# yezhen17/3DIoUMatch

Hardware: AMD Instinct MI355X
Metric: scenes/sec train-step (ScanNet 40k pts, 256 proposals) (higher is better)
Workload: dtype f32

## Files before the change

3dioumatch_amd/_lib.py:

```python
import ctypes
import os

_HERE = os.path.dirname(os.path.abspath(__file__))
LIB_PATH = os.path.join(_HERE, "lib3dioumatch_hip%s.so" % os.environ.get("PN2_LIB_SUFFIX", ""))

_c_int, _c_float, _vp, _sz = ctypes.c_int, ctypes.c_float, ctypes.c_void_p, ctypes.c_size_t


class MlpOperand(ctypes.Structure):
    _fields_ = [("mode", _c_int), ("x", _vp), ("dz", _vp), ("scale", _vp), ("shift", _vp), ("mean", _vp),
                ("invstd", _vp), ("coef", _vp), ("argmax", _vp), ("ns", _c_int), ("groups", _c_int),
                ("lin_w", _vp)]


_op = ctypes.POINTER(MlpOperand)

_SIGNATURES = {
    "pn2_furthest_point_sampling": [_c_int, _c_int, _c_int, _vp, _vp, _vp, _vp],
    "pn2_furthest_point_sampling_ws": [_c_int, _c_int, _c_int, _vp, _vp, _vp, _sz, _vp],
    "pn2_fps_workspace_bytes": [_c_int, _c_int, _c_int],
    "pn2_gather_points": [_c_int, _c_int, _c_int, _c_int, _vp, _vp, _vp, _vp],
    "pn2_gather_points_grad": [_c_int, _c_int, _c_int, _c_int, _vp, _vp, _vp, _vp],
    "pn2_ball_query": [_c_int, _c_int, _c_int, _c_float, _c_int, _vp, _vp, _vp, _vp, _sz, _vp],
    "pn2_ball_query_workspace_bytes": [_c_int, _c_int, _c_int, _c_int],
# ... 84 lines not shown
    "mlp_wgrad_first4_from_gated": [_c_int] + [_vp] * 9,
    "mlp_first4_moments_doubles": [],
    "mlp_first4_moments": [_c_int, _c_int, _vp, _vp, _vp],
    "mlp_first4_bn": [_vp, ctypes.c_double, _vp, _vp, _vp, _c_float, _c_float, _vp, _vp, _vp, _vp, _vp, _vp,
                      _vp],
    "mlp_gemm_backward_fused_supported": [_c_int, _c_int, _c_int, _c_int, _c_int, _c_int, _c_int],
    "mlp_gemm_backward_fused_workspace_floats": [_c_int, _c_int, _c_int, _c_int],
    "mlp_gemm_backward_fused": [_c_int] * 4 + [_vp, _op, _op] + [_vp] * 5,
    "mlp_gemm_backward_fused_stats_parts": [_c_int, _c_int, _c_int, _c_int],
    "mlp_bn_backward_finalize": [_c_int, _c_int, ctypes.c_double, _c_int, _vp, _vp, _vp, _vp, _vp, _vp,
                                 _vp],
    "mlp_gemm_backward_small_supported": [_c_int, _c_int, _c_int, _c_int, _c_int, _c_int],
    "mlp_weight_image_elems": [_c_int, _c_int],
    "mlp_weight_images_build": [_c_int, _vp, _vp, _vp, _vp, _vp, _vp],
    "mlp_gemm_image_supported": [_c_int, _c_int],
    "mlp_gemm_backward_small": [_c_int] * 4 + [_vp, _vp, _op, _op] + [_vp] * 4,
    "mlp_pregather_supported": [_c_int, _c_int, _c_int, _c_int, _c_int],
    "mlp_pregather_pack": [_c_int, _c_int, _c_int, _c_int, ctypes.c_float, _vp, _vp, _vp, _vp, _vp],
    "mlp_pregather_unpack_grad": [_c_int, _c_int, _c_int, _c_int, _vp, _vp, _vp],
    "mlp_pregather_forward": [_c_int, _c_int, _c_int, _c_int, _c_int, _vp, _vp, _vp, _vp, _vp],
    "mlp_pregather_backward": [_c_int] * 5 + [_op, _vp, _vp, _vp],
    "mlp_defer_weight_reductions": [_c_int],
    "mlp_flush_weight_reductions": [],
    "lhs_nms3d_aabb": [_c_int, _c_int, _vp, _vp, _vp, _vp, _vp, ctypes.c_double, _c_int, _c_int, _vp,
                       _vp],
    "lhs_nms_aabb_masked": [_c_int, _c_int, _vp, _vp, _vp, _vp, _vp, ctypes.c_double, _c_int, _c_int,
                            _c_int, _vp, _vp, _vp],
    "lhs_box_point_count": [_c_int] * 4 + [_vp] * 6,
    "votenet_decode_scores": [_c_int] * 5 + [_vp] * 13,
    "votenet_decode_scores_grad": [_c_int] * 5 + [_vp] * 13,
    "lhs_pseudo_select": [_vp, _vp],
    "lhs_pseudo_finish": [_vp, _vp],
    "lhs_pseudo_stats": [_vp, _vp],
    "lhs_pseudo_stats_workspace_bytes": [_c_int, _c_int],
    "lhs_nms_samecls": [_c_int, _c_int, _vp, _vp, _vp, _vp, _vp, ctypes.c_double, _c_int, _vp, _vp],
    "iou3d_boxes_overlap_bev": [_c_int, _vp, _c_int, _vp, _vp, _vp],
    "iou3d_boxes_iou_bev": [_c_int, _vp, _c_int, _vp, _vp, _vp],
    "iou3d_boxes_iou3d": [_c_int, _vp, _c_int, _vp, _vp, _vp],
    "iou3d_scene_best_iou3d": [_c_int, _c_int, _vp, _c_int, _vp, _vp, _vp, _vp],
    "votenet_loss_decode": [_vp, _vp],
    "votenet_loss_forward_backward": [_vp, _vp],
    "votenet_loss_scratch_floats": [_vp],
    "votenet_eval_loss_decode": [_vp, _vp],
    "votenet_eval_loss": [_vp, _vp, _vp, _vp],
    "votenet_bbox_jitter": [_c_int, _c_int, _c_int, _c_int] + [_vp] * 15,
    "votenet_gridconv_points": [_c_int, _c_int, _c_int, _vp, _vp, _vp, _vp, _vp, _vp, _vp],
# ... 64 lines not shown
```

3dioumatch_amd/csrc/mlp_bwd_fused.hip:

```cpp
#include "common.h"
#include "mlp_operand.h"
#include "mlp_bwd_x6.h"

#ifndef MLP_LIN4_OCC
#define MLP_LIN4_OCC 1
#endif

namespace {

template <int MB, int KB, int KBD, int NB, int PMODE, int QMODE, int OCC, bool STATS, bool DGRAD = true,
          bool X6 = false>
__global__ void __launch_bounds__(256, OCC)
gemm_bwd_fused_kernel(int k_total, int r, int total_chunks, int chunks_per_cloud, int xyz,
                      OperandB opp, OperandB opq, const float *__restrict__ w,
                      float *__restrict__ dq, float *__restrict__ part,
                      float *__restrict__ stats_part) {
  constexpr int M = 32 * MB, KP = 32 * KB, TN = 32 * NB;
  constexpr int LDP = M + 1, LDQ = KP + 1;
  constexpr int TPR = TN / 16;
  constexpr int RPP = 256 / TPR;
  constexpr int PP = (M + RPP - 1) / RPP, QP = (KP + RPP - 1) / RPP;
  constexpr int WMB = MB >= 4 ? MB / 4 : 1;
  constexpr int WKB = MB >= 4 ? KB : KB * MB / 4;
  static_assert(MB >= 4 ? MB % 4 == 0 : (MB == 2 && KB % 2 == 0), "dW blocks must split over 4 waves");
// ... 496 lines not shown
      const int colk = kb * 32 + l31;
      if (colk >= k_total) continue;
#pragma unroll
      for (int q = 0; q < 16; ++q) {
        const int row = mb * 32 + (q & 3) + 8 * (q >> 2) + 4 * lhi;
        out[(size_t)row * k_total + colk] = accW[i][j][q];
      }
    }
  }
}

struct FusedShape { int m, k, xyz, tn, occ; };

bool fused_shape(int m, int k, FusedShape *s) {
  static const FusedShape table[] = {
      {64, 64, 0, 64, 2}, {128, 64, 0, 64, 1}, {128, 128, 0, 32, 2},
      {256, 128, 0, 32, 1}, {128, 131, 3, 32, 1}, {128, 259, 3, 32, 1},
  };
  for (const FusedShape &t : table)
    if (t.m == m && t.k == k) { *s = t; return true; }
  return false;
}

int fused_cus() {
  static int cus = 0;
  if (!cus) {
    int dev = 0;
    if (hipGetDevice(&dev) != hipSuccess ||
        hipDeviceGetAttribute(&cus, hipDeviceAttributeMultiprocessorCount, dev) != hipSuccess || cus <= 0)
      cus = 256;
  }
  return cus;
}

int fused_workgroups(const FusedShape &s, long long total_chunks) {
  long long g = (long long)fused_cus() * s.occ;
  if (g > total_chunks / 8) g = total_chunks / 8;
  return (int)(g < 1 ? 1 : g);
}

}

#define MLP_API extern "C" __attribute__((visibility("default")))

MLP_API int mlp_gemm_backward_fused_supported(int b, int m, int k, int r, int pmode, int qmode,
                                              int ns) {
  FusedShape s;
  if (b <= 0 || r <= 0 || !fused_shape(m, k, &s)) return 0;
  if (r % s.tn != 0 || (long long)b * (r / s.tn) < 64) return 0;
  if (pmode != OP_DY && pmode != OP_POOLDY) return 0;
  if (pmode == OP_POOLDY && (ns <= 0 || ns % 16 != 0 || r % ns != 0 || (ns % s.tn != 0 && s.tn % ns != 0)))
    return 0;
  if (qmode == OP_LIN4) return m == 64 && k == 64 && pmode == OP_DY;
  const bool first = s.xyz != 0;
  if (first != (qmode == OP_DIRECT)) return 0;
  if (qmode != OP_DIRECT && qmode != OP_BNRELU) return 0;
  const bool pooled_only = (m == 128 && k == 64) || (m == 256 && k == 128);
  const bool either = m == 128 && k == 128;
  if (!either && pooled_only != (pmode == OP_POOLDY)) return 0;
  return 1;
}

MLP_API int mlp_gemm_backward_fused_stats_parts(int b, int m, int k, int r) {
  FusedShape s;
  const int gx = mlp_bwd_x6_workgroups(b, m, k, r, fused_cus());
  if (gx > 0) return gx;
  if (!fused_shape(m, k, &s) || k != 64 || r % s.tn != 0) return 0;
  return fused_workgroups(s, (long long)b * (r / s.tn)) * 2;
}

MLP_API size_t mlp_gemm_backward_fused_workspace_floats(int b, int m, int k, int r) {
  FusedShape s;
  if (!fused_shape(m, k, &s) || r % s.tn != 0) return 0;
  const long long g0 = fused_workgroups(s, (long long)b * (r / s.tn));
  const long long g1 = mlp_bwd_x6_workgroups(b, m, k, r, fused_cus());
  return (size_t)(g0 > g1 ? g0 : g1) * m * k;
}

MLP_API int mlp_gemm_backward_fused(int b, int m, int k, int r, const float *w, const MlpOperand *dy,
                                    const MlpOperand *x, float *dq, float *dw, float *workspace,
                                    float *stats_part, void *stream_) {
  if (b <= 0 || m <= 0 || k <= 0 || r <= 0) return 0;
  OperandB P, Q;
  int orc = operand_from_abi(dy, op_bit(OP_DY) | op_bit(OP_POOLDY), r, &P);
  if (!orc) orc = operand_from_abi(x, op_bit(OP_DIRECT) | op_bit(OP_BNRELU) | op_bit(OP_LIN4), r, &Q);
  if (orc) return orc;
  const int pmode = dy->mode, qmode = x->mode;
  if (qmode != OP_DIRECT && (!Q.mean || !Q.invstd)) return (int)hipErrorInvalidValue;
  if (!mlp_gemm_backward_fused_supported(b, m, k, r, pmode, qmode, P.ns)) return (int)hipErrorInvalidValue;
  FusedShape s;
  fused_shape(m, k, &s);
  if (dq == nullptr && !(m == 128 && k == 259)) return (int)hipErrorInvalidValue;
  hipStream_t stream = (hipStream_t)stream_;
  const int cpc = r / s.tn;
  const int total = b * cpc;
  const int g = fused_workgroups(s, total);
  {
    int gx = 0;
    const int rcx = mlp_bwd_x6_try(b, m, k, r, pmode, qmode, P, Q, w, dq, workspace,
                                   qmode == OP_BNRELU ? stats_part : nullptr, fused_cus(), &gx, stream);
    if (rcx > 0) return rcx;
    if (rcx == 0) return mlp_reduce_weight_partials(m * k, gx, workspace, dw, stream);
  }
  if (k != 64) stats_part = nullptr;
#define FUSED_X(MB, KB, KBD, NB, PM, QM, OCC, ST, X6)                                           \
  hipLaunchKernelGGL((gemm_bwd_fused_kernel<MB, KB, KBD, NB, PM, QM, OCC, ST, true, X6>), dim3(g), \
                     dim3(256), 0, stream, k, r, total, cpc, s.xyz, P, Q, w, dq, workspace,     \
                     stats_part)
#define FUSED(MB, KB, KBD, NB, PM, QM, OCC, ST) FUSED_X(MB, KB, KBD, NB, PM, QM, OCC, ST, true)
#define FUSED_F32(MB, KB, KBD, NB, PM, QM, OCC, ST) FUSED_X(MB, KB, KBD, NB, PM, QM, OCC, ST, false)
  if (m == 64 && k == 64 && qmode == OP_LIN4) FUSED(2, 2, 2, 2, OP_DY, OP_LIN4, MLP_LIN4_OCC, true);
  else if (m == 64 && k == 64) FUSED(2, 2, 2, 2, OP_DY, OP_BNRELU, 2, true);
  else if (m == 128 && k == 64) FUSED(4, 2, 2, 2, OP_POOLDY, OP_BNRELU, 1, true);
  else if (m == 256 && k == 128) FUSED(8, 4, 4, 1, OP_POOLDY, OP_BNRELU, 1, false);
  else if (m == 128 && k == 131) FUSED(4, 5, 4, 1, OP_DY, OP_DIRECT, 1, false);
  else if (dq != nullptr) FUSED_F32(4, 9, 8, 1, OP_DY, OP_DIRECT, 1, false);
  else
    hipLaunchKernelGGL((gemm_bwd_fused_kernel<4, 9, 8, 1, OP_DY, OP_DIRECT, 1, false, false, true>), dim3(g),
                       dim3(256), 0, stream, k, r, total, cpc, s.xyz, P, Q, w, dq, workspace, stats_part);
#undef FUSED_F32
#undef FUSED
#undef FUSED_X
  int rc = pn2_launch_status();
// ... 4 lines not shown
```

3dioumatch_amd/csrc/mlp_bwd_x6.h:

```cpp
#pragma once
#include "common.h"
#include "mlp_operand.h"
#include <type_traits>

namespace {

typedef short bf16x4 __attribute__((ext_vector_type(4)));

#if defined(BWDX6_ABL) && BWDX6_ABL == 2
#define mfma_x6(ACC, A, B) do { (ACC)[0] += __builtin_bit_cast(float, (int)(A).hi[0] + (int)(B).hi[0] + (int)(A).mid[1] + (int)(B).mid[1] + (int)(A).lo[2] + (int)(B).lo[2]); } while (0)
#endif

__device__ __forceinline__ bf16x4 lds_read_tr(const char *p) {
  return __builtin_amdgcn_ds_read_tr16_b64_v4i16(
      (__attribute__((address_space(3))) bf16x4 *)(__attribute__((address_space(3))) char *)p);
}

__device__ __forceinline__ float x6_half_wave_sum(float v) {
#define HW_STEP(CTRL, RM) v += __builtin_bit_cast(float, __builtin_amdgcn_update_dpp(0, __builtin_bit_cast(int, v), CTRL, RM, 0xf, false))
  HW_STEP(0xB1, 0xf);
  HW_STEP(0x4E, 0xf);
  HW_STEP(0x141, 0xf);
  HW_STEP(0x140, 0xf);
  HW_STEP(0x142, 0xa);
#undef HW_STEP
// ... 377 lines not shown
  extern __shared__ __attribute__((aligned(16))) char lds[];
  const int wave = __builtin_amdgcn_readfirstlane((int)threadIdx.x >> 6);
  if (STATS) {
    constexpr int KP = 32 * KB;
    constexpr int RCOFF = 2 * (3 * (32 * MB + KP) * 80 + KP * 144);
    float4 *rc = reinterpret_cast<float4 *>(lds + RCOFF);
    for (int t = threadIdx.x; t < KP; t += 512)
      rc[t] = t < k_total ? make_float4(opq.scale[t], opq.shift[t], opq.mean[t], opq.invstd[t])
                          : make_float4(0.f, 0.f, 0.f, 0.f);
  }
  if (wave < 4) {
    gemm_bwd_x6_role<MB, KB, KBD, PMODE, QMODE, STATS, true>(
        k_total, r, total_chunks, chunks_per_cloud, xyz, opp, opq, w, dq, part, stats_part, lds,
        (int)threadIdx.x, wave);
  } else {
    gemm_bwd_x6_role<MB, KB, KBD, PMODE, QMODE, STATS, false>(
        k_total, r, total_chunks, chunks_per_cloud, xyz, opp, opq, w, dq, part, stats_part, lds,
        (int)threadIdx.x - 256, wave - 4);
  }
}

}

static int mlp_bwd_x6_workgroups(int b, int m, int k, int r, int cus) {
  if (!(m == 128 && k == 128) || r % 32 != 0 || b <= 0) return 0;
  const long long total = (long long)b * (r / 32);
  long long g = cus;
  if (g > total / 8) g = total / 8;
  return (int)(g < 1 ? 1 : g);
}

static int mlp_bwd_x6_try(int b, int m, int k, int r, int pmode, int qmode, const OperandB &P,
                          const OperandB &Q, const float *w, float *dq, float *part,
                          float *stats_part, int cus, int *workgroups, hipStream_t stream) {
  const int g = mlp_bwd_x6_workgroups(b, m, k, r, cus);
  if (g == 0 || qmode != OP_BNRELU || dq == nullptr) return -1;
  const int total_chunks = b * (r / 32), chunks_per_cloud = r / 32;
  *workgroups = g;
  constexpr int RP = 80;
#define BWDX6(MB, KB, KBD, PM, QM, ST)                                                              \
  do {                                                                                              \
    const size_t lds_bytes = 2 * (3 * (size_t)(m + k) * RP + (ST ? (size_t)k * 144 : 0)) +         \
                             (ST ? (size_t)k * 16 : 0);                                             \
    auto kern = gemm_bwd_x6_kernel<MB, KB, KBD, PM, QM, ST>;                                        \
    static bool attr_set = false;                                                                   \
    if (!attr_set) {                                                                                \
      (void)hipFuncSetAttribute(reinterpret_cast<const void *>(kern),                               \
                                hipFuncAttributeMaxDynamicSharedMemorySize, (int)lds_bytes);        \
      attr_set = true;                                                                              \
    }                                                                                               \
    hipLaunchKernelGGL(kern, dim3(g), dim3(512), lds_bytes, stream, k, r, total_chunks,             \
                       chunks_per_cloud, 0, P, Q, w, dq, part, stats_part);                         \
  } while (0)
  const bool st = stats_part != nullptr;
  if (pmode == OP_DY && st) BWDX6(4, 4, 4, OP_DY, OP_BNRELU, true);
  else if (pmode == OP_DY) BWDX6(4, 4, 4, OP_DY, OP_BNRELU, false);
  else if (pmode == OP_POOLDY && st) BWDX6(4, 4, 4, OP_POOLDY, OP_BNRELU, true);
  else if (pmode == OP_POOLDY) BWDX6(4, 4, 4, OP_POOLDY, OP_BNRELU, false);
// ... 5 lines not shown
```

3dioumatch_amd/csrc/mlp_chain.hip:

```cpp
#include "common.h"
#include "mlp_operand.h"
#include <mutex>
#include <set>
#include <type_traits>

namespace {

struct ChainArgs {
  int r;
  int tiles_per_cloud;
  const float *x4;
  const char *wimg;
  const float *sc2, *sh2;
  const float *gamma3;
  float *y2;
  float *y3;
  float *pairs;
  float *ext;
  size_t ext_plane;
};

constexpr int kChainK = 64;

template <int R>
// ... 315 lines not shown
    const float mo = __shfl_xor(mh, 32, kWave), qo = __shfl_xor(qh, 32, kWave);
    if (h == 0) {
      const float dlt = mo - mh;
      wstat[wave * (32 * CB) + 32 * j + l31] = make_float2(0.5f * (mh + mo), (qh + qo) + 0.5f * n_half * dlt * dlt);
    }
  }
  __syncthreads();
  if (tid < 32 * CB) {
    float mean = 0.f, m2 = 0.f;
#pragma unroll
    for (int w = 0; w < 4; ++w) { mean += wstat[w * (32 * CB) + tid].x; m2 += wstat[w * (32 * CB) + tid].y; }
    mean *= 0.25f;
#pragma unroll
    for (int w = 0; w < 4; ++w) {
      const float d = wstat[w * (32 * CB) + tid].x - mean;
      m2 = __fmaf_rn(2.f * n_half * d, d, m2);
    }
    float *dst = a.pairs + ((size_t)blockIdx.x * (32 * CB) + tid) * 2;
    dst[0] = mean;
    dst[1] = m2;
  }
}

int chain_cus() {
  static int cus = 0;
  if (!cus) {
    int dev = 0;
    if (hipGetDevice(&dev) != hipSuccess ||
        hipDeviceGetAttribute(&cus, hipDeviceAttributeMultiprocessorCount, dev) != hipSuccess || cus <= 0)
      cus = 256;
  }
  return cus;
}

bool chain_shape_ok(int b, int r, int ns) {
  return b > 0 && r > 0 && r % (32 * 4 * kTilesPerWave) == 0 && (ns == 16 || ns == 32 || ns == 64) &&
         r % ns == 0 && (long long)b * (r / 32) < (1LL << 30);
}

int chain_workgroups(int b, int r) { return (int)((long long)b * (r / 32) / (4 * kTilesPerWave)); }

template <typename Kern>
void chain_launch(Kern kern, int wgs, size_t lds_bytes, hipStream_t stream, const ChainArgs &args) {
  static std::mutex mu;
  static std::set<const void *> done;
  {
    std::lock_guard<std::mutex> lock(mu);
    if (done.insert(reinterpret_cast<const void *>(kern)).second)
      (void)hipFuncSetAttribute(reinterpret_cast<const void *>(kern),
                                hipFuncAttributeMaxDynamicSharedMemorySize, (int)lds_bytes);
  }
  hipLaunchKernelGGL(kern, dim3(wgs), dim3(256), lds_bytes, stream, args);
}

__device__ __forceinline__ double chain_wave_sum(double v) {
#pragma unroll
  for (int off = 1; off < kWave; off <<= 1) {
// ... 127 lines not shown
```

3dioumatch_amd/csrc/mlp_eval_pool.hip:

```cpp
#include "common.h"
#include "mlp_operand.h"
#include <mutex>
#include <set>

namespace {

template <int K, int R>
__device__ __forceinline__ int ev_off(int term, int t, int h, int row) {
  return (((term * (K / 16) + t) * 2 + h) * R + row) * 16;
}

__device__ __forceinline__ Split3 ev_frag(const char *p, int term_stride) {
  Split3 s;
  s.hi = *reinterpret_cast<const bf16x8 *>(p);
  s.mid = *reinterpret_cast<const bf16x8 *>(p + term_stride);
  s.lo = *reinterpret_cast<const bf16x8 *>(p + 2 * term_stride);
  return s;
}

template <int NB, bool TFORM, bool FIRST = false>
__device__ __forceinline__ void ev_mfma6(f32x16 (&acc)[NB], const Split3 &s, const Split3 (&w)[NB]) {
  const f32x16 zero = {0.f, 0.f, 0.f, 0.f, 0.f, 0.f, 0.f, 0.f, 0.f, 0.f, 0.f, 0.f, 0.f, 0.f, 0.f, 0.f};
#define EV_STEP(WT, ST, C0)                                                                        \
  _Pragma("unroll") for (int i = 0; i < NB; ++i)                                                  \
// ... 339 lines not shown
      ev_pool<HB, NS>(acc2, c2tab, HB * hf, l31, best, 0);
      if constexpr (TPG == 2) {
        float *slot = carry + ((wave * HALVES + hf) * HB) * 64 + lane;
        if (p == 0) {
#pragma unroll
          for (int j = 0; j < HB; ++j) slot[64 * j] = best[j][0];
          continue;
        }
#pragma unroll
        for (int j = 0; j < HB; ++j) best[j][0] = fmaxf(best[j][0], slot[64 * j]);
      }
      ev_pool_store<HB, NS>(best, a.out, (size_t)b * M2 + 32 * HB * hf, groups, g0, l31, h);
    }
  }
}

bool stored_shape_ok(int b, int c_in, int c_mid, int c_out, int m, int ns) {
  if (b <= 0 || m <= 0 || c_in != 128 || c_mid != 128 || !(c_out == 128 || c_out == 256)) return false;
  if (!(ns == 16 || ns == 32 || ns == 64)) return false;
  const long long r = (long long)m * ns;
  return r % 32 == 0 && (long long)b * r * 128 < (1LL << 31) * 4LL && (long long)b * r < (1LL << 31);
}

int eval_cus() {
  static int cus = 0;
  if (!cus) {
    int dev = 0;
    if (hipGetDevice(&dev) != hipSuccess ||
        hipDeviceGetAttribute(&cus, hipDeviceAttributeMultiprocessorCount, dev) != hipSuccess || cus <= 0)
      cus = 256;
  }
  return cus;
}

int stored_tiles_per_wave(int b, int m, int ns) {
  const long long total_tiles = (long long)b * m * ns / 32;
  return (ns == 64 || total_tiles >= 4 * 2 * 2 * eval_cus()) ? 2 : 1;
}

template <typename Kern, typename Args>
void eval_launch(Kern kern, int wgs, size_t lds_bytes, hipStream_t stream, const Args &args) {
  static std::mutex mu;
  static std::set<const void *> done;
  {
    std::lock_guard<std::mutex> lock(mu);
    if (done.insert(reinterpret_cast<const void *>(kern)).second)
      (void)hipFuncSetAttribute(reinterpret_cast<const void *>(kern),
                                hipFuncAttributeMaxDynamicSharedMemorySize, (int)lds_bytes);
  }
  hipLaunchKernelGGL(kern, dim3(wgs), dim3(256), lds_bytes, stream, args);
}

bool misaligned(const void *p) { return (reinterpret_cast<size_t>(p) & 15) != 0; }

}

#define MLP_API extern "C" __attribute__((visibility("default")))

MLP_API int mlp_eval_lin4_supported(int b, int c_in, int c_mid, int c_out, int m, int ns) {
  return (c_in == 4 && c_mid == 64 && c_out == 128 && lin4_shape_ok(b, m, ns)) ? 1 : 0;
// ... 66 lines not shown
```

3dioumatch_amd/csrc/mlp_pool_fwd256.hip:

```cpp
#include "common.h"
#include "mlp_operand.h"
#include <stdlib.h>
#include <mutex>
#include <type_traits>

namespace {

typedef short f_bf16x4 __attribute__((ext_vector_type(4)));

__device__ __forceinline__ f_bf16x4 f_lds_read_tr(const char *p) {
  return __builtin_amdgcn_ds_read_tr16_b64_v4i16(
      (__attribute__((address_space(3))) f_bf16x4 *)(__attribute__((address_space(3))) char *)p);
}

constexpr int kFM = 256, kFK = 128, kFTN = 32;
constexpr int kFRP = kFTN * 2;
constexpr int kFIMG = kFK * kFRP;
constexpr int kFBUF = 3 * kFIMG;
constexpr int kFTP = 32 * 144;

struct PoolFwdArgs {
  int r, chunks_per_cloud, total_tiles, groups;
  const float *w;
  const float *x;
// ... 276 lines not shown
      switch (3 * s + 1) {
        PF_CASE(1); PF_CASE(4); PF_CASE(7); PF_CASE(10); PF_CASE(13); PF_CASE(16); PF_CASE(19);
      }
      PF_MM(hi, mid) PF_MM1(hi, hi)
      switch (3 * s + 2) {
        PF_CASE(2); PF_CASE(5); PF_CASE(8); PF_CASE(11); PF_CASE(14); PF_CASE(20);
      }
#undef PF_CASE
#undef PF_MM
#undef PF_MM1
      if (s == 3) __syncthreads();
    }
    cur = nxt;
#pragma unroll
    for (int j = 0; j < 8; ++j) pv[j] = f_f32x2{acc[2 * j], acc[2 * j + 1]} + f_f32x2{acc1[2 * j], acc1[2 * j + 1]};
  }
  ce = c_hi - 1;
  real = true;
  PF_PIECE(9); PF_PIECE(10); PF_PIECE(11); PF_PIECE(12); PF_PIECE(13); PF_PIECE(14); PF_PIECE(15);
  PF_PIECE(16); PF_PIECE(18); PF_PIECE(19); PF_PIECE(20); PF_PIECE(21);
#undef PF_PIECE
}

int pool_fwd256_cus() {
  static int cus = 0;
  if (!cus) {
    int dev = 0;
    if (hipGetDevice(&dev) != hipSuccess ||
        hipDeviceGetAttribute(&cus, hipDeviceAttributeMultiprocessorCount, dev) != hipSuccess || cus <= 0)
      cus = 256;
  }
  return cus;
}

}

int mlp_pool_fwd256_supported(int b, int m, int k, int r, int ns, const float *w, const MlpOperand &x) {
  const char *env = getenv("MLP_POOL_FWD256");
  const bool off = env && atoi(env) == 0;
  if (off || b <= 0 || m != kFM || k != kFK || r <= 0 || r % 256 != 0) return 0;
  if ((ns != 16 && ns != 32) || r % ns != 0) return 0;
  return ((reinterpret_cast<size_t>(w) | reinterpret_cast<size_t>(x.x)) & 15) == 0 ? 1 : 0;
}

int mlp_pool_fwd256_launch(int b, int r, int ns, const float *w, const MlpOperand &x, const float *gamma,
                           float *y, float *pairs, float *ext, hipStream_t stream) {
  if (!w || !x.x || !x.scale || !x.shift || !gamma || !pairs || !ext || (ns != 16 && ns != 32) || b <= 0 || r <= 0 ||
      r % 256 != 0)
    return (int)hipErrorInvalidValue;
  PoolFwdArgs a = {};
  a.r = r; a.chunks_per_cloud = r / kFTN; a.total_tiles = b * (r / 64); a.groups = r / ns;
  a.w = w; a.x = x.x; a.sc = x.scale; a.sh = x.shift; a.gamma = gamma; a.pairs = pairs; a.ext = ext; a.y = y;
  a.ext_plane = (size_t)b * kFM * (size_t)(r / ns);
  int grid = pool_fwd256_cus();
  if (grid > a.total_tiles / 2) grid = a.total_tiles / 2;
  const size_t kLds = 3 * (size_t)kFBUF + (y != nullptr ? 8 * (size_t)kFTP : 0);
  constexpr size_t kLdsMax = 3 * (size_t)kFBUF + 8 * (size_t)kFTP;
  static std::mutex mu;
  static bool attr_set = false;
  {
    std::lock_guard<std::mutex> lock(mu);
    if (!attr_set) {
      (void)hipFuncSetAttribute(reinterpret_cast<const void *>(pool_fwd256_kernel<16, false>),
                                hipFuncAttributeMaxDynamicSharedMemorySize, (int)kLdsMax);
      (void)hipFuncSetAttribute(reinterpret_cast<const void *>(pool_fwd256_kernel<32, false>),
                                hipFuncAttributeMaxDynamicSharedMemorySize, (int)kLdsMax);
      (void)hipFuncSetAttribute(reinterpret_cast<const void *>(pool_fwd256_kernel<16, true>),
                                hipFuncAttributeMaxDynamicSharedMemorySize, (int)kLdsMax);
      (void)hipFuncSetAttribute(reinterpret_cast<const void *>(pool_fwd256_kernel<32, true>),
                                hipFuncAttributeMaxDynamicSharedMemorySize, (int)kLdsMax);
      attr_set = true;
    }
  }
  if (y != nullptr) {
    if (ns == 16) hipLaunchKernelGGL((pool_fwd256_kernel<16, true>), dim3(grid), dim3(512), kLds, stream, a);
    else hipLaunchKernelGGL((pool_fwd256_kernel<32, true>), dim3(grid), dim3(512), kLds, stream, a);
  } else {
    if (ns == 16) hipLaunchKernelGGL((pool_fwd256_kernel<16, false>), dim3(grid), dim3(512), kLds, stream, a);
// ... 5 lines not shown
```

3dioumatch_amd/csrc/mlp_pool_gram.hip:

```cpp
#include "common.h"
#include "mlp_operand.h"
#include <mutex>
#include <type_traits>

namespace {

typedef short g_bf16x4 __attribute__((ext_vector_type(4)));

__device__ __forceinline__ g_bf16x4 g_lds_read_tr(const char *p) {
  return __builtin_amdgcn_ds_read_tr16_b64_v4i16(
      (__attribute__((address_space(3))) g_bf16x4 *)(__attribute__((address_space(3))) char *)p);
}

constexpr int kGM = 128, kGK = 64;

__global__ void __launch_bounds__(256)
pool_gram_prep_kernel(const float *__restrict__ w3, const float *__restrict__ coef3,
                      const float *__restrict__ mean3, const float *__restrict__ invstd3,
                      float *__restrict__ qp, float *__restrict__ m3, float *__restrict__ v) {
  __shared__ float q[kGM], p[kGM];
  const int tid = threadIdx.x;
  if (tid < kGM) {
    const float a = coef3[tid * 3], c1 = coef3[tid * 3 + 1], c2 = coef3[tid * 3 + 2];
    const float t = invstd3[tid] * c2;
// ... 404 lines not shown
  for (; p < parts; p += 8) s += (double)src[(size_t)p * stride];
  red[sl][threadIdx.x & 31] = s;
  __syncthreads();
  if (sl == 0) {
    double t = 0.0;
#pragma unroll
    for (int q = 0; q < 8; ++q) t += red[q][threadIdx.x];
    sums[e] = t;
  }
}

__global__ void __launch_bounds__(256)
pool_gram_dw_kernel(const float *__restrict__ w3, const float *__restrict__ qp,
                    const double *__restrict__ sums, float *__restrict__ dw) {
  const int e = blockIdx.x * 256 + threadIdx.x;
  if (e >= kGM * kGK) return;
  const int c = e >> 6, k = e & 63;
  const double *c2 = sums, *s2 = sums + kGK * kGK, *rr = s2 + kGK;
  double acc = 0.0;
  for (int k2 = 0; k2 < kGK; ++k2) acc += (double)w3[c * kGK + k2] * c2[k2 * kGK + k];
  dw[e] = (float)((double)qp[c * 2] * acc + (double)qp[c * 2 + 1] * s2[k] + rr[e]);
}

int gram_cus() {
  static int cus = 0;
  if (!cus) {
    int dev = 0;
    if (hipGetDevice(&dev) != hipSuccess ||
        hipDeviceGetAttribute(&cus, hipDeviceAttributeMultiprocessorCount, dev) != hipSuccess || cus <= 0)
      cus = 256;
  }
  return cus;
}

int gram_workgroups(int b, int r) {
  const long long total = (long long)b * (r / 32);
  long long g = gram_cus();
  if (g > total / 8) g = total / 8;
  return (int)(g < 1 ? 1 : g);
}

constexpr size_t kGramLds = 2 * (3 * (128 + 64) * 80 + 64 * 144) + 64 * 16 + 64 * 4;

}

#define MLP_API extern "C" __attribute__((visibility("default")))

static bool gram_covers(int b, int r, int ns) {
  if (b <= 0 || r <= 0 || r % 32 != 0) return false;
  if ((ns != 16 && ns != 32 && ns != 64) || r % ns != 0) return false;
  return (long long)b * (r / 32) >= 64;
}
static bool is128(int m, int k) { return m == kGM && k == kGK; }
static bool is256(int m, int k) { return m == 256 && k == 128; }

MLP_API int mlp_pool_gram_supported(int b, int m, int k, int r, int ns) {
  if (is128(m, k)) return gram_covers(b, r, ns) ? 1 : 0;
  return is256(m, k) && mlp_pool_gram256_supported(b, r, ns) ? 1 : 0;
}

MLP_API int mlp_pool_gram_parts(int b, int m, int k, int r) {
  if (is128(m, k)) return gram_workgroups(b, r);
  return is256(m, k) ? mlp_pool_gram256_parts(b, r) : 0;
// ... 53 lines not shown
```

3dioumatch_amd/csrc/mlp_pool_gram256.hip:

```cpp
#include "common.h"
#include "mlp_operand.h"
#include <stdlib.h>
#include <mutex>
#include <type_traits>

namespace {

typedef short h_bf16x4 __attribute__((ext_vector_type(4)));
typedef unsigned h_u32x4 __attribute__((ext_vector_type(4)));

__device__ __forceinline__ h_bf16x4 h_lds_read_tr(const char *p) {
  return __builtin_amdgcn_ds_read_tr16_b64_v4i16(
      (__attribute__((address_space(3))) h_bf16x4 *)(__attribute__((address_space(3))) char *)p);
}

constexpr int kHM = 256, kHK = 128, kHTN = 32;
constexpr int kHRP = kHTN * 2 + 16;
constexpr int kHQIMG = kHK * kHRP;
constexpr int kHRAWP = (kHTN + 4) * 4;
constexpr int kHRAW = kHK * kHRAWP;
constexpr int kHSP = kHM * 2 + 16;
constexpr int kHSIMG = kHTN * kHSP;

__global__ void __launch_bounds__(256)
// ... 638 lines not shown
                       const double *__restrict__ sums, float *__restrict__ dw) {
  __shared__ double part[kHK];
  const int c = blockIdx.x, k = threadIdx.x & (kHK - 1), half = threadIdx.x >> 7;
  const double *c2 = sums, *s2 = sums + kHK * kHK, *rr = s2 + kHK;
  double acc = 0.0;
  for (int k0 = half * (kHK / 2); k0 < (half + 1) * (kHK / 2); k0 += 16) {
    double g[16];
    float w[16];
#pragma unroll
    for (int j = 0; j < 16; ++j) {
      const int k2 = k0 + j;
      g[j] = (k2 >> 5) <= (k >> 5) ? c2[k2 * kHK + k] : c2[k * kHK + k2];
      w[j] = w3[c * kHK + k2];
    }
#pragma unroll
    for (int j = 0; j < 16; ++j) acc += (double)w[j] * g[j];
  }
  if (half == 1) part[k] = acc;
  __syncthreads();
  if (half == 0)
    dw[c * kHK + k] = (float)((double)qp[c * 2] * (acc + part[k]) + (double)qp[c * 2 + 1] * s2[k] + rr[c * kHK + k]);
}

int gram256_cus() {
  static int cus = 0;
  if (!cus) {
    int dev = 0;
    if (hipGetDevice(&dev) != hipSuccess ||
        hipDeviceGetAttribute(&cus, hipDeviceAttributeMultiprocessorCount, dev) != hipSuccess || cus <= 0)
      cus = 256;
  }
  return cus;
}

int gram256_workgroups(int b, int r, int least) {
  const long long total = (long long)b * (r / 32);
  long long g = gram256_cus();
  if (g > total / least) g = total / least;
  return (int)(g < 1 ? 1 : g);
}
constexpr int kDgradLeast = 8, kWgradLeast = 16;

constexpr size_t kDgradLds = 2 * (3 * (size_t)kHQIMG + kHRAW) + 3 * (size_t)(kHSIMG + kHSP) + kHK * 16 + kHK * 4;
constexpr size_t kWgradLds = 2 * 3 * (size_t)kHQIMG;
static_assert(kDgradLds <= 160 * 1024, "LDS of the data-gradient pass");

}

static bool gram256_covers(int b, int r, int ns) {
  return b > 0 && r > 0 && r % 32 == 0 && (ns == 16 || ns == 32) && r % ns == 0;
}

bool mlp_pool_gram256_supported(int b, int r, int ns) {
  const long long least = getenv("MLP_POOL_GRAM256_MIN_CHUNKS") ? atoll(getenv("MLP_POOL_GRAM256_MIN_CHUNKS")) : 4096;
  return gram256_covers(b, r, ns) && (long long)b * (r / 32) >= least;
}

int mlp_pool_gram256_parts(int b, int r) { return gram256_workgroups(b, r, kDgradLeast); }
size_t mlp_pool_gram256_workspace_floats(int b, int r, int ns) {
  const size_t g = (size_t)gram256_workgroups(b, r, kWgradLeast);
  const size_t groups = ns > 0 ? (size_t)(r / ns) : 0;
  return 512 + 16384 + 128 + (size_t)b * groups * kHM * 2 + g * (size_t)kHSums + 2 * (size_t)kHSums + 16;
// ... 54 lines not shown
```

3dioumatch_amd/dropin/pointnet2/_mlp_ext.py:

```python
import contextlib
import ctypes
import os

import torch

from pointnet2._ext import _L, _lib, _stream

SMALL_BWD_DY_COLS = 4096


def _f32c(t, name):
    if t.dtype != torch.float32 or not t.is_contiguous() or not t.is_cuda:
        raise RuntimeError("%s must be a contiguous float32 GPU tensor" % name)


def _ws(y, b, c, r):
    n = int(_lib.mlp_bn_workspace_floats(b, c, r))
    return torch.empty(max(n, 1), dtype=torch.float32, device=y.device)


def new_tickets(channels, device):
    return torch.zeros(max(int(channels), 1), dtype=torch.int32, device=device)


# ... 352 lines not shown
    return small[0], small[1], small[2:]


def gemm_dgrad(w, dy=None, fly=None, pooled=None):
    m, k = w.shape
    _f32c(w, "w")
    op = _grad_operand(dy, fly, pooled)
    src = op.tensors["x"]
    b = src.shape[0]
    r = src.numel() // (b * m)
    dx = torch.empty((b, k) + tuple(src.shape[2:]), dtype=torch.float32, device=src.device)
    with torch.cuda.device(src.device):
        _L.check(_lib.mlp_gemm_dgrad(b, m, k, r, w.data_ptr(), ctypes.byref(op), dx.data_ptr(),
                                     _stream(src)), "mlp_gemm_dgrad")
    return dx


_queued_workspaces = None


def _keep_until_flush(*tensors):
    if _queued_workspaces is not None:
        _queued_workspaces.extend(t for t in tensors if t is not None)


@contextlib.contextmanager
def deferred_weight_reductions(enabled=True):
    global _queued_workspaces
    if not enabled or _queued_workspaces is not None:
        yield
        return
    _queued_workspaces = []
    _L.check(_lib.mlp_defer_weight_reductions(1), "mlp_defer_weight_reductions")
    try:
        yield
    finally:
        held, device = _queued_workspaces, None
        if held:
            device = held[0].device
        try:
            if device is not None:
                with torch.cuda.device(device):
                    rc = _lib.mlp_defer_weight_reductions(0)
            else:
                rc = _lib.mlp_defer_weight_reductions(0)
        finally:
# ... 417 lines not shown
```

3dioumatch_amd/votenet/step.py:

```python
import os
import weakref
import sys

import numpy as np
import torch

from pointnet2._mlp_ext import deferred_weight_reductions
from pointnet2.pytorch_utils import deferred_bn_counters, zero_grads_none

from .detector import VoteNet
from .data import BOX_LABEL_KEYS
from .losses import get_labeled_loss


def build_detector(cfg, num_proposal=256, input_feature_dim=1, sampling="seed_fps", seed=0):
    torch.manual_seed(seed)
    return VoteNet(cfg.num_class, cfg.num_heading_bin, cfg.num_size_cluster, cfg.mean_size_arr,
                   cfg, input_feature_dim=input_feature_dim, num_proposal=num_proposal,
                   sampling=sampling)


def wrap_ddp(net, device, world_size):
    if world_size <= 1:
        return net
# ... 439 lines not shown
    def _refresh_lr(self):
        if self._lr_scalar is None:
            return
        lr = self.optimizer.param_groups[0]["lr"]
        if torch.is_tensor(lr):
            self._lr_scalar.copy_(lr, non_blocking=True)
        else:
            self._lr_scalar.fill_(float(lr))

    def _before_apply(self):
        self.global_step += 1
        self._refresh_lr()

    def side_stream(self):
        if self.device.type != "cuda":
            return None
        if self._side is None:
            key = (self.device.type, self.device.index)
            if key not in _SIDE_STREAMS:
                _SIDE_STREAMS[key] = torch.cuda.Stream(device=self.device)
            self._side = _SIDE_STREAMS[key]
        return self._side

    def prefetch_geometry(self, batch):
        if self.device.type != "cuda":
            batch["geometry"] = self._compute_geometry(batch)
            return
        self.side_stream()
        main = torch.cuda.current_stream(self.device)
        if self.graphs and self._ensure_captured(batch):
            slot = self._slots[self._turn]
            self._turn ^= 1
            self._side.wait_stream(main)
            with torch.cuda.stream(self._side):
                self._stage(slot, batch)
                slot["graph"].replay()
                slot["ready"].record(self._side)
            self._token += 1
            slot["token"] = self._token
            batch["geometry"] = slot["geometry"]
            batch["_staged"] = (slot, self._token)
            return
        self._side.wait_stream(main)
        with torch.cuda.stream(self._side):
            geometry = self._compute_geometry(batch)
            done = torch.cuda.Event()
            done.record(self._side)
        for t in geometry.values():
            if torch.is_tensor(t):
                t.record_stream(main)
        batch["geometry"] = geometry
# ... 5 lines not shown
            return None
        host = batch.get("supervised_mask_host")
        if host is None:
            ref, version, cached = self._mask_cache
            if ref is None or ref() is not mask or version != mask._version:
                cached = tuple(int(v) for v in mask.detach().cpu().reshape(-1).tolist())
                self._mask_cache = (weakref.ref(mask), mask._version, cached)
            host = cached
        return tuple(int(v) != 0 for v in host)

    def _signature(self, batch):
        shapes = tuple(sorted((k, tuple(v.shape), str(v.dtype)) for k, v in _tensor_items(batch).items()))
        return shapes, self._mask_facts(batch)

    def _stage(self, slot, batch):
        src = _tensor_items(batch)
        torch._foreach_copy_([slot["inputs"][k] for k in self._keys], [src[k] for k in self._keys])

    def _ensure_captured(self, batch):
        sig = self._signature(batch)
        if self._captured == sig:
            return True
        try:
            self._capture(batch, sig)
            return True
        except Exception as err:
            if not self.graphs_fallback:
                raise
            sys.stderr.write("SupervisedStep: HIP graph capture failed (%s: %s); running the "
                             "step eagerly (graphs_fallback=True)\n" % (type(err).__name__, err))
            torch.cuda.synchronize(self.device)
            self.graphs = False
            self._captured = None
            return False

    def _capture(self, batch, sig):
        dev = self.device
        self._refresh_lr()
        torch.cuda.synchronize(dev)
        src = _tensor_items(batch)
        src.pop("supervised_inds", None)
        self._keys = sorted(src)
        self._slots = [{"inputs": {k: src[k].clone(memory_format=torch.contiguous_format)
                                   for k in self._keys}, "token": -1,
                        "ready": torch.cuda.Event()} for _ in range(2)]
        self._turn = 0
        self._cur = {k: src[k].clone(memory_format=torch.contiguous_format) for k in self._keys}
# ... 164 lines not shown
                 unlabeled_loss_weight=2.0, ema_decay=0.999, dataset="scannet", config_dict=None,
                 graphs_fallback=False, meter=False, guard=False, clip_grad_norm=None):
        super().__init__(cfg, device, world_size=world_size, num_proposal=num_proposal, lr=lr,
                         seed=seed, graphs=graphs, graphs_fallback=graphs_fallback, meter=meter,
                         guard=guard, clip_grad_norm=clip_grad_norm)
        from .losses_unlabeled import default_config_dict
        self.teacher = build_detector(cfg, num_proposal=num_proposal, seed=seed).to(device).train()
        for p in self.teacher.parameters():
            p.requires_grad_(False)
        self.flat_teacher = flatten_parameters(self.teacher).data
        self.flat_teacher.copy_(self.flat_params.data)
        if self.guarded:
            self._home_guard_state([self.net, self.teacher])
        self.unlabeled_loss_weight = unlabeled_loss_weight
        self.ema_decay = ema_decay
        self.config_dict = config_dict or default_config_dict(cfg, dataset=dataset)
        self._ema_weight = torch.zeros((), device=device)
        self._teacher_stream = None
        self._teacher_replay = None
        self._gt = None


    batch_chains = os.environ.get("STEP_SEMI_ONE_CHAIN", "1") != "0"

    def _compute_geometry(self, inputs):
        pc, ema = inputs["point_clouds"], inputs["ema_point_clouds"]
        if self.batch_chains and pc.shape[1:] == ema.shape[1:] and pc.dtype == ema.dtype:
            nb = pc.shape[0]
            both = self.net.compute_geometry({"point_clouds": torch.cat([pc, ema], dim=0)})
            geometry = {}
            for k, v in both.items():
                if not torch.is_tensor(v) or v.dim() == 0 or v.shape[0] != nb + ema.shape[0]:
                    raise RuntimeError("geometry entry %r is not batched along dim 0" % k)
                geometry[k] = v[:nb]
                geometry["ema_" + k] = v[nb:]
            return geometry
        geometry = dict(self.net.compute_geometry(inputs))
        teacher = self.teacher.compute_geometry({"point_clouds": ema})
        geometry.update({"ema_" + k: v for k, v in teacher.items()})
        return geometry

    def _host_info(self, src):
        mask = src["supervised_mask"]
        labeled = int(torch.count_nonzero(mask))
        if not bool((mask[:labeled] != 0).all()):
            raise ValueError("labeled scenes must come first in the batch (train.py:321-325)")
# ... 227 lines not shown
```

include/mlp_hip.h:

```cpp
#ifndef MLP_HIP_H
#define MLP_HIP_H

#include <stddef.h>

#ifdef __cplusplus
extern "C" {
#endif

size_t mlp_bn_workspace_floats(int b, int c, int r);


int mlp_bn_train_stats(int b, int c, int r, const float *y, const float *gamma, const float *beta,
                       float eps, float momentum, float *running_mean, float *running_var,
                       float *mean, float *invstd, float *scale, float *shift, float *workspace,
                       int *tickets, void *stream);

int mlp_bn_eval_coeff(int c, const float *gamma, const float *beta, float eps,
                      const float *running_mean, const float *running_var, float *mean,
                      float *invstd, float *scale, float *shift, void *stream);

int mlp_bn_relu_apply(int b, int c, int r, const float *y, const float *scale, const float *shift,
                      float *z, void *stream);

int mlp_bn_relu_pool(int b, int c, int m, int ns, const float *y, const float *scale,
// ... 77 lines not shown
                             const float *shift, float *pooled, int *argmax, float *ymax,
                             void *stream);

int mlp_gemm_backward_fused_supported(int b, int m, int k, int r, int pmode, int qmode, int ns);
size_t mlp_gemm_backward_fused_workspace_floats(int b, int m, int k, int r);
int mlp_gemm_backward_fused(int b, int m, int k, int r, const float *w, const MlpOperand *dy,
                            const MlpOperand *x, float *dq, float *dw, float *workspace,
                            float *stats_part, void *stream);
int mlp_gemm_backward_small_supported(int b, int m, int k, int r, int pmode, int qmode);
int mlp_gemm_backward_small(int b, int m, int k, int r, const float *w, const void *img_t,
                            const MlpOperand *dy, const MlpOperand *x, float *dq, float *dw,
                            float *workspace, void *stream);
size_t mlp_weight_image_elems(int m, int k);
int mlp_weight_images_build(int n, const void *const *w, const int *m, const int *k,
                            void *const *img, void *const *img_t, void *stream);
int mlp_gemm_image_supported(int b, int r);
int mlp_gemm_backward_fused_stats_parts(int b, int m, int k, int r);
int mlp_bn_backward_finalize(int c, int parts, double count, int training, const float *partial,
                             const float *gamma, const float *invstd, float *dgamma, float *dbeta,
                             float *coef, void *stream);
int mlp_defer_weight_reductions(int on);
int mlp_flush_weight_reductions(void);

int mlp_pregather_supported(int b, int c, int n, int m, int ns);
int mlp_pregather_pack(int b, int n, int m, int c, float s, const float *xyz, const float *new_xyz,
                       const float *features, float *src_ext, void *stream);
int mlp_pregather_unpack_grad(int b, int n, int m, int c, const float *dsrc_ext, float *dfeatures,
                              void *stream);
int mlp_pregather_forward(int b, int c, int n, int m, int ns, const float *z_ext, const int *idx,
                          float *y, float *pairs, void *stream);
int mlp_pregather_backward(int b, int c, int n, int m, int ns, const MlpOperand *dy,
                           const unsigned *inverse, float *dz_ext, void *stream);

int mlp_first4_moments_doubles(void);
int mlp_first4_moments(int b, int r, const float *x, double *moments, void *stream);
int mlp_first4_bn(const double *moments, double count, const float *w, const float *gamma,
                  const float *beta, float eps, float momentum, float *running_mean,
                  float *running_var, float *mean, float *invstd, float *scale, float *shift,
                  void *stream);
size_t mlp_wgrad_first4_workspace_bytes(int b, int r);
int mlp_wgrad_first4(int b, int r, const float *w, const float *x, const float *dz,
                     const float *scale, const float *shift, const float *mean, const float *invstd,
                     const float *coef, const double *moments, float *dw, void *workspace,
                     void *stream);
int mlp_wgrad_first4_from_gated(int parts, const float *gpart, const float *w, const float *mean,
                                const float *invstd, const float *coef, const double *moments,
// ... 20 lines not shown
```

Measured before the change: 1421.

## Reserve CUs for side-stream geometry chain when sizing persistent grids

Moves the per-file CU-count helpers into one shared persistent-grid module, which can subtract a reserved CU count when sizing persistent workgroup grids. During graph capture, the step reserves CUs in whole shader-engine rows, scaled to the cloud count. This applies only to the order-free pool forward kernel, so the geometry chain on the side stream can run alongside it without being starved. The risk is that the main-stream kernel gets fewer workgroups and takes longer.

New measurement: 1430 (median of 6 runs). No clear change (+0.7%).

```diff
diff --git a/3dioumatch_amd/_lib.py b/3dioumatch_amd/_lib.py
--- a/3dioumatch_amd/_lib.py
+++ b/3dioumatch_amd/_lib.py
@@ -130,6 +130,11 @@
     "mlp_pregather_backward": [_c_int] * 5 + [_op, _vp, _vp, _vp],
     "mlp_defer_weight_reductions": [_c_int],
     "mlp_flush_weight_reductions": [],
+    "mlp_persistent_cus": [],
+    "mlp_persistent_reserve": [_c_int],
+    "mlp_persistent_reserve_clouds": [_c_int],
+    "mlp_persistent_reserved_cus": [_c_int],
+    "mlp_persistent_workgroups": [_c_int, ctypes.c_longlong, _c_int, _c_int],
     "lhs_nms3d_aabb": [_c_int, _c_int, _vp, _vp, _vp, _vp, _vp, ctypes.c_double, _c_int, _c_int, _vp,
                        _vp],
     "lhs_nms_aabb_masked": [_c_int, _c_int, _vp, _vp, _vp, _vp, _vp, ctypes.c_double, _c_int, _c_int,
diff --git a/3dioumatch_amd/csrc/mlp_bwd_fused.hip b/3dioumatch_amd/csrc/mlp_bwd_fused.hip
--- a/3dioumatch_amd/csrc/mlp_bwd_fused.hip
+++ b/3dioumatch_amd/csrc/mlp_bwd_fused.hip
@@ -542,21 +542,8 @@
   return false;
 }
 
-int fused_cus() {
-  static int cus = 0;
-  if (!cus) {
-    int dev = 0;
-    if (hipGetDevice(&dev) != hipSuccess ||
-        hipDeviceGetAttribute(&cus, hipDeviceAttributeMultiprocessorCount, dev) != hipSuccess || cus <= 0)
-      cus = 256;
-  }
-  return cus;
-}
-
 int fused_workgroups(const FusedShape &s, long long total_chunks) {
-  long long g = (long long)fused_cus() * s.occ;
-  if (g > total_chunks / 8) g = total_chunks / 8;
-  return (int)(g < 1 ? 1 : g);
+  return persistent_workgroups(s.occ, total_chunks, 8);
 }
 
 }
@@ -583,7 +570,7 @@
 
 MLP_API int mlp_gemm_backward_fused_stats_parts(int b, int m, int k, int r) {
   FusedShape s;
-  const int gx = mlp_bwd_x6_workgroups(b, m, k, r, fused_cus());
+  const int gx = mlp_bwd_x6_workgroups(b, m, k, r);
   if (gx > 0) return gx;
   if (!fused_shape(m, k, &s) || k != 64 || r % s.tn != 0) return 0;
   return fused_workgroups(s, (long long)b * (r / s.tn)) * 2;
@@ -593,7 +580,7 @@
   FusedShape s;
   if (!fused_shape(m, k, &s) || r % s.tn != 0) return 0;
   const long long g0 = fused_workgroups(s, (long long)b * (r / s.tn));
-  const long long g1 = mlp_bwd_x6_workgroups(b, m, k, r, fused_cus());
+  const long long g1 = mlp_bwd_x6_workgroups(b, m, k, r);
   return (size_t)(g0 > g1 ? g0 : g1) * m * k;
 }
 
@@ -618,7 +605,7 @@
   {
     int gx = 0;
     const int rcx = mlp_bwd_x6_try(b, m, k, r, pmode, qmode, P, Q, w, dq, workspace,
-                                   qmode == OP_BNRELU ? stats_part : nullptr, fused_cus(), &gx, stream);
+                                   qmode == OP_BNRELU ? stats_part : nullptr, &gx, stream);
     if (rcx > 0) return rcx;
     if (rcx == 0) return mlp_reduce_weight_partials(m * k, gx, workspace, dw, stream);
   }
diff --git a/3dioumatch_amd/csrc/mlp_bwd_x6.h b/3dioumatch_amd/csrc/mlp_bwd_x6.h
--- a/3dioumatch_amd/csrc/mlp_bwd_x6.h
+++ b/3dioumatch_amd/csrc/mlp_bwd_x6.h
@@ -1,6 +1,7 @@
 #pragma once
 #include "common.h"
 #include "mlp_operand.h"
+#include "persistent_grid.h"
 #include <type_traits>
 
 namespace {
@@ -424,18 +425,15 @@
 
 }
 
-static int mlp_bwd_x6_workgroups(int b, int m, int k, int r, int cus) {
+static int mlp_bwd_x6_workgroups(int b, int m, int k, int r) {
   if (!(m == 128 && k == 128) || r % 32 != 0 || b <= 0) return 0;
-  const long long total = (long long)b * (r / 32);
-  long long g = cus;
-  if (g > total / 8) g = total / 8;
-  return (int)(g < 1 ? 1 : g);
+  return persistent_workgroups(1, (long long)b * (r / 32), 8);
 }
 
 static int mlp_bwd_x6_try(int b, int m, int k, int r, int pmode, int qmode, const OperandB &P,
                           const OperandB &Q, const float *w, float *dq, float *part,
-                          float *stats_part, int cus, int *workgroups, hipStream_t stream) {
-  const int g = mlp_bwd_x6_workgroups(b, m, k, r, cus);
+                          float *stats_part, int *workgroups, hipStream_t stream) {
+  const int g = mlp_bwd_x6_workgroups(b, m, k, r);
   if (g == 0 || qmode != OP_BNRELU || dq == nullptr) return -1;
   const int total_chunks = b * (r / 32), chunks_per_cloud = r / 32;
   *workgroups = g;
diff --git a/3dioumatch_amd/csrc/mlp_chain.hip b/3dioumatch_amd/csrc/mlp_chain.hip
--- a/3dioumatch_amd/csrc/mlp_chain.hip
+++ b/3dioumatch_amd/csrc/mlp_chain.hip
@@ -361,17 +361,6 @@
   }
 }
 
-int chain_cus() {
-  static int cus = 0;
-  if (!cus) {
-    int dev = 0;
-    if (hipGetDevice(&dev) != hipSuccess ||
-        hipDeviceGetAttribute(&cus, hipDeviceAttributeMultiprocessorCount, dev) != hipSuccess || cus <= 0)
-      cus = 256;
-  }
-  return cus;
-}
-
 bool chain_shape_ok(int b, int r, int ns) {
   return b > 0 && r > 0 && r % (32 * 4 * kTilesPerWave) == 0 && (ns == 16 || ns == 32 || ns == 64) &&
          r % ns == 0 && (long long)b * (r / 32) < (1LL << 30);
diff --git a/3dioumatch_amd/csrc/mlp_eval_pool.hip b/3dioumatch_amd/csrc/mlp_eval_pool.hip
--- a/3dioumatch_amd/csrc/mlp_eval_pool.hip
+++ b/3dioumatch_amd/csrc/mlp_eval_pool.hip
@@ -1,5 +1,6 @@
 #include "common.h"
 #include "mlp_operand.h"
+#include "persistent_grid.h"
 #include <mutex>
 #include <set>
 
@@ -385,20 +386,9 @@
   return r % 32 == 0 && (long long)b * r * 128 < (1LL << 31) * 4LL && (long long)b * r < (1LL << 31);
 }
 
-int eval_cus() {
-  static int cus = 0;
-  if (!cus) {
-    int dev = 0;
-    if (hipGetDevice(&dev) != hipSuccess ||
-        hipDeviceGetAttribute(&cus, hipDeviceAttributeMultiprocessorCount, dev) != hipSuccess || cus <= 0)
-      cus = 256;
-  }
-  return cus;
-}
-
 int stored_tiles_per_wave(int b, int m, int ns) {
   const long long total_tiles = (long long)b * m * ns / 32;
-  return (ns == 64 || total_tiles >= 4 * 2 * 2 * eval_cus()) ? 2 : 1;
+  return (ns == 64 || total_tiles >= 4 * 2 * 2 * persistent_cus()) ? 2 : 1;
 }
 
 template <typename Kern, typename Args>
diff --git a/3dioumatch_amd/csrc/mlp_pool_fwd256.hip b/3dioumatch_amd/csrc/mlp_pool_fwd256.hip
--- a/3dioumatch_amd/csrc/mlp_pool_fwd256.hip
+++ b/3dioumatch_amd/csrc/mlp_pool_fwd256.hip
@@ -1,5 +1,6 @@
 #include "common.h"
 #include "mlp_operand.h"
+#include "persistent_grid.h"
 #include <stdlib.h>
 #include <mutex>
 #include <type_traits>
@@ -322,17 +323,6 @@
 #undef PF_PIECE
 }
 
-int pool_fwd256_cus() {
-  static int cus = 0;
-  if (!cus) {
-    int dev = 0;
-    if (hipGetDevice(&dev) != hipSuccess ||
-        hipDeviceGetAttribute(&cus, hipDeviceAttributeMultiprocessorCount, dev) != hipSuccess || cus <= 0)
-      cus = 256;
-  }
-  return cus;
-}
-
 }
 
 int mlp_pool_fwd256_supported(int b, int m, int k, int r, int ns, const float *w, const MlpOperand &x) {
@@ -352,8 +342,7 @@
   a.r = r; a.chunks_per_cloud = r / kFTN; a.total_tiles = b * (r / 64); a.groups = r / ns;
   a.w = w; a.x = x.x; a.sc = x.scale; a.sh = x.shift; a.gamma = gamma; a.pairs = pairs; a.ext = ext; a.y = y;
   a.ext_plane = (size_t)b * kFM * (size_t)(r / ns);
-  int grid = pool_fwd256_cus();
-  if (grid > a.total_tiles / 2) grid = a.total_tiles / 2;
+  const int grid = persistent_workgroups(1, a.total_tiles, 2, true);
   const size_t kLds = 3 * (size_t)kFBUF + (y != nullptr ? 8 * (size_t)kFTP : 0);
   constexpr size_t kLdsMax = 3 * (size_t)kFBUF + 8 * (size_t)kFTP;
   static std::mutex mu;
diff --git a/3dioumatch_amd/csrc/mlp_pool_gram.hip b/3dioumatch_amd/csrc/mlp_pool_gram.hip
--- a/3dioumatch_amd/csrc/mlp_pool_gram.hip
+++ b/3dioumatch_amd/csrc/mlp_pool_gram.hip
@@ -1,5 +1,6 @@
 #include "common.h"
 #include "mlp_operand.h"
+#include "persistent_grid.h"
 #include <mutex>
 #include <type_traits>
 
@@ -450,23 +451,7 @@
   dw[e] = (float)((double)qp[c * 2] * acc + (double)qp[c * 2 + 1] * s2[k] + rr[e]);
 }
 
-int gram_cus() {
-  static int cus = 0;
-  if (!cus) {
-    int dev = 0;
-    if (hipGetDevice(&dev) != hipSuccess ||
-        hipDeviceGetAttribute(&cus, hipDeviceAttributeMultiprocessorCount, dev) != hipSuccess || cus <= 0)
-      cus = 256;
-  }
-  return cus;
-}
-
-int gram_workgroups(int b, int r) {
-  const long long total = (long long)b * (r / 32);
-  long long g = gram_cus();
-  if (g > total / 8) g = total / 8;
-  return (int)(g < 1 ? 1 : g);
-}
+int gram_workgroups(int b, int r) { return persistent_workgroups(1, (long long)b * (r / 32), 8); }
 
 constexpr size_t kGramLds = 2 * (3 * (128 + 64) * 80 + 64 * 144) + 64 * 16 + 64 * 4;
 
diff --git a/3dioumatch_amd/csrc/mlp_pool_gram256.hip b/3dioumatch_amd/csrc/mlp_pool_gram256.hip
--- a/3dioumatch_amd/csrc/mlp_pool_gram256.hip
+++ b/3dioumatch_amd/csrc/mlp_pool_gram256.hip
@@ -1,5 +1,6 @@
 #include "common.h"
 #include "mlp_operand.h"
+#include "persistent_grid.h"
 #include <stdlib.h>
 #include <mutex>
 #include <type_traits>
@@ -684,22 +685,8 @@
     dw[c * kHK + k] = (float)((double)qp[c * 2] * (acc + part[k]) + (double)qp[c * 2 + 1] * s2[k] + rr[c * kHK + k]);
 }
 
-int gram256_cus() {
-  static int cus = 0;
-  if (!cus) {
-    int dev = 0;
-    if (hipGetDevice(&dev) != hipSuccess ||
-        hipDeviceGetAttribute(&cus, hipDeviceAttributeMultiprocessorCount, dev) != hipSuccess || cus <= 0)
-      cus = 256;
-  }
-  return cus;
-}
-
 int gram256_workgroups(int b, int r, int least) {
-  const long long total = (long long)b * (r / 32);
-  long long g = gram256_cus();
-  if (g > total / least) g = total / least;
-  return (int)(g < 1 ? 1 : g);
+  return persistent_workgroups(1, (long long)b * (r / 32), least);
 }
 constexpr int kDgradLeast = 8, kWgradLeast = 16;
 
diff --git a/3dioumatch_amd/csrc/persistent_grid.h b/3dioumatch_amd/csrc/persistent_grid.h
--- /dev/null
+++ b/3dioumatch_amd/csrc/persistent_grid.h
@@ -0,0 +1,7 @@
+#pragma once
+
+constexpr int kPersistentShaderEngines = 32;
+
+int persistent_cus();
+int persistent_reserved_cus(bool order_free);
+int persistent_workgroups(int per_cu, long long total_units, long long least_units, bool order_free = false);
diff --git a/3dioumatch_amd/csrc/persistent_grid.hip b/3dioumatch_amd/csrc/persistent_grid.hip
--- /dev/null
+++ b/3dioumatch_amd/csrc/persistent_grid.hip
@@ -0,0 +1,64 @@
+#include "common.h"
+#include "persistent_grid.h"
+#include "../../include/mlp_hip.h"
+#include <stdlib.h>
+#include <atomic>
+
+namespace {
+
+std::atomic<int> g_reserve{0};
+std::atomic<int> g_reserve_free{0};
+
+}
+
+int persistent_cus() {
+  static std::atomic<int> cached{0};
+  int cus = cached.load(std::memory_order_relaxed);
+  if (!cus) {
+    int dev = 0;
+    if (hipGetDevice(&dev) != hipSuccess ||
+        hipDeviceGetAttribute(&cus, hipDeviceAttributeMultiprocessorCount, dev) != hipSuccess || cus <= 0)
+      cus = 256;
+    cached.store(cus, std::memory_order_relaxed);
+  }
+  return cus;
+}
+
+int persistent_reserved_cus(bool order_free) {
+  const char *env = getenv("MLP_RESERVED_CUS");
+  long long r = g_reserve.load(std::memory_order_relaxed);
+  if (order_free && g_reserve_free.load(std::memory_order_relaxed) > r) r = g_reserve_free.load(std::memory_order_relaxed);
+  if (env && *env) r = atoll(env);
+  const int cus = persistent_cus();
+  if (r < 0) r = 0;
+  if (r > cus - 1) r = cus - 1;
+  return (int)r;
+}
+
+int persistent_workgroups(int per_cu, long long total_units, long long least_units, bool order_free) {
+  long long g = (long long)(persistent_cus() - persistent_reserved_cus(order_free)) * per_cu;
+  if (g > total_units / least_units) g = total_units / least_units;
+  return (int)(g < 1 ? 1 : g);
+}
+
+#define MLP_API extern "C" __attribute__((visibility("default")))
+
+MLP_API int mlp_persistent_cus() { return persistent_cus(); }
+
+MLP_API int mlp_persistent_reserved_cus(int order_free) { return persistent_reserved_cus(order_free != 0); }
+
+MLP_API int mlp_persistent_reserve(int cus) {
+  return g_reserve.exchange(cus < 0 ? 0 : cus, std::memory_order_relaxed);
+}
+
+MLP_API int mlp_persistent_reserve_clouds(int clouds) {
+  if (clouds < 0) clouds = 0;
+  const long long rows = ((long long)clouds + kPersistentShaderEngines - 1) / kPersistentShaderEngines;
+  const long long cus = rows * kPersistentShaderEngines;
+  return g_reserve_free.exchange(cus > (1 << 20) ? (1 << 20) : (int)cus, std::memory_order_relaxed);
+}
+
+MLP_API int mlp_persistent_workgroups(int per_cu, long long total_units, int least_units, int order_free) {
+  if (per_cu <= 0 || total_units < 0 || least_units <= 0) return 0;
+  return persistent_workgroups(per_cu, total_units, least_units, order_free != 0);
+}
diff --git a/3dioumatch_amd/dropin/pointnet2/_mlp_ext.py b/3dioumatch_amd/dropin/pointnet2/_mlp_ext.py
--- a/3dioumatch_amd/dropin/pointnet2/_mlp_ext.py
+++ b/3dioumatch_amd/dropin/pointnet2/_mlp_ext.py
@@ -398,6 +398,18 @@
 def _keep_until_flush(*tensors):
     if _queued_workspaces is not None:
         _queued_workspaces.extend(t for t in tensors if t is not None)
+
+
+def persistent_cus():
+    return int(_lib.mlp_persistent_cus())
+
+
+def persistent_reserve(cus):
+    return int(_lib.mlp_persistent_reserve(int(cus)))
+
+
+def persistent_reserve_clouds(clouds):
+    return int(_lib.mlp_persistent_reserve_clouds(int(clouds)))
 
 
 @contextlib.contextmanager
diff --git a/3dioumatch_amd/votenet/step.py b/3dioumatch_amd/votenet/step.py
--- a/3dioumatch_amd/votenet/step.py
+++ b/3dioumatch_amd/votenet/step.py
@@ -485,11 +485,21 @@
             self._side = _SIDE_STREAMS[key]
         return self._side
 
+    _chain_reserve = None
+
+    def _chain_clouds(self, batch):
+        return int(batch["point_clouds"].shape[0])
+
+    def _reserve_for_chain(self, batch):
+        if self._chain_reserve is None and self._captured is None:
+            self._chain_reserve = self._chain_clouds(batch)
+
     def prefetch_geometry(self, batch):
         if self.device.type != "cuda":
             batch["geometry"] = self._compute_geometry(batch)
             return
         self.side_stream()
+        self._reserve_for_chain(batch)
         main = torch.cuda.current_stream(self.device)
         if self.graphs and self._ensure_captured(batch):
             slot = self._slots[self._turn]
@@ -541,7 +551,15 @@
         if self._captured == sig:
             return True
         try:
-            self._capture(batch, sig)
+            if self._chain_reserve is None:
+                self._capture(batch, sig)
+            else:
+                from pointnet2 import _mlp_ext as K
+                before = K.persistent_reserve_clouds(self._chain_reserve)
+                try:
+                    self._capture(batch, sig)
+                finally:
+                    K.persistent_reserve_clouds(before)
             return True
         except Exception as err:
             if not self.graphs_fallback:
@@ -752,6 +770,9 @@
 
 
     batch_chains = os.environ.get("STEP_SEMI_ONE_CHAIN", "1") != "0"
+
+    def _chain_clouds(self, batch):
+        return int(batch["point_clouds"].shape[0]) + int(batch["ema_point_clouds"].shape[0])
 
     def _compute_geometry(self, inputs):
         pc, ema = inputs["point_clouds"], inputs["ema_point_clouds"]
diff --git a/include/mlp_hip.h b/include/mlp_hip.h
--- a/include/mlp_hip.h
+++ b/include/mlp_hip.h
@@ -123,6 +123,12 @@
 int mlp_defer_weight_reductions(int on);
 int mlp_flush_weight_reductions(void);
 
+int mlp_persistent_cus(void);
+int mlp_persistent_reserve(int cus);
+int mlp_persistent_reserve_clouds(int clouds);
+int mlp_persistent_reserved_cus(int order_free);
+int mlp_persistent_workgroups(int per_cu, long long total_units, int least_units, int order_free);
+
 int mlp_pregather_supported(int b, int c, int n, int m, int ns);
 int mlp_pregather_pack(int b, int n, int m, int c, float s, const float *xyz, const float *new_xyz,
                        const float *features, float *src_ext, void *stream);
```
